# trevor-m/cuda-pathtrace

Measured on AMD Instinct MI355X. Metric: Msamples/s, 9-sphere Cornell box 1024x1024x1024spp, higher is better.
Workload: dtype f32+f64

## Files before the change

### cuda-pathtrace_amd/__init__.py

```python
import ctypes
import os

import numpy as np

_HERE = os.path.dirname(os.path.abspath(__file__))
LIB_PATH = os.environ.get("PT_LIB_OVERRIDE") or os.path.join(_HERE, "libptcore.so")
LAB_LIB_PATH = os.path.join(_HERE, "libptcore_lab.so")
INCLUDE_DIR = os.path.join(os.path.dirname(_HERE), "include")

if not os.path.exists(LIB_PATH):
    raise ImportError(
        f"{LIB_PATH} is missing: build it with `make -C cuda-pathtrace_amd/csrc` "
        "(or __graft_entry__.build()); there is no fallback implementation"
    )

RNG_XORWOW = 0
RNG_PHILOX = 1
CHANNELS = 14

SPHERE_DTYPE = np.dtype([("radius", "<f4"), ("pos", "<f4", 3), ("emission", "<f4", 3), ("color", "<f4", 3)])
assert SPHERE_DTYPE.itemsize == 40


class PtError(RuntimeError):
# ... 115 lines not shown
    "pt_filter_opts_default": (None, [_vp]),
    "pt_filter_create": (ctypes.c_int, [ctypes.c_int, ctypes.c_int, _vp, ctypes.POINTER(_vp)]),
    "pt_filter_destroy": (ctypes.c_int, [_vp]),
    "pt_filter_reserve_frames": (ctypes.c_int, [_vp, ctypes.c_int]),
    "pt_filter_workspace_bytes": (ctypes.c_int, [_vp, ctypes.POINTER(ctypes.c_uint64)]),
    "pt_filter_enqueue": (ctypes.c_int, [_vp, _vp, _vp, ctypes.c_int, _vp, _vp]),
    "pt_filter_run": (ctypes.c_int, [_vp, _vp, _vp, ctypes.c_int, _vp, _fp]),
    "pt_filter_enqueue_frames": (ctypes.c_int, [_vp, ctypes.c_int, _vp, ctypes.c_size_t, _vp, ctypes.c_size_t, ctypes.c_int, _vp]),
    "pt_filter_run_frames": (ctypes.c_int, [_vp, ctypes.c_int, _vp, ctypes.c_size_t, _vp, ctypes.c_size_t, ctypes.c_int, _fp]),
    "pt_progressive_create": (ctypes.c_int, [_vp, ctypes.POINTER(_vp)]),
    "pt_progressive_reset": (ctypes.c_int, [_vp]),
    "pt_progressive_enqueue": (ctypes.c_int, [_vp, ctypes.c_int, _vp, _vp, ctypes.c_int, _fp, _fp, _vp]),
    "pt_progressive_render": (ctypes.c_int, [_vp, ctypes.c_int, _vp, _vp, ctypes.c_int, _fp, _fp, _fp]),
    "pt_progressive_samples": (ctypes.c_int, [_vp, ctypes.POINTER(ctypes.c_int64)]),
    "pt_progressive_variant": (ctypes.c_int, [_vp, ctypes.c_int, ctypes.POINTER(ctypes.c_int)]),
    "pt_progressive_destroy": (ctypes.c_int, [_vp]),
    "pt_progressive_set_adaptive": (ctypes.c_int, [_vp, _vp]),
    "pt_progressive_active": (ctypes.c_int, [_vp, ctypes.POINTER(ctypes.c_int64)]),
    "pt_progressive_counts": (ctypes.c_int, [_vp, _vp, _vp]),
}
LAB_ABI = {
    "pt_debug_unary_map": (ctypes.c_int, [ctypes.c_int, _vp, _vp, ctypes.c_size_t]),
    "pt_debug_unary_compare": (ctypes.c_int, [ctypes.c_int, ctypes.c_int, ctypes.c_uint32, ctypes.c_uint64,
                                              ctypes.POINTER(ctypes.c_uint64), ctypes.POINTER(ctypes.c_uint32)]),
    "pt_debug_div_compare": (ctypes.c_int, [ctypes.c_uint32, ctypes.c_uint32, ctypes.c_uint32, ctypes.c_uint64,
                                            ctypes.POINTER(ctypes.c_uint64), ctypes.POINTER(ctypes.c_uint32),
                                            ctypes.POINTER(ctypes.c_uint32)]),
    "pt_debug_grid_header": (ctypes.c_int, [_vp, ctypes.c_int, ctypes.POINTER(ctypes.c_uint32)]),
    "pt_debug_grid_image": (ctypes.c_int, [_vp, ctypes.c_int, _fp, ctypes.c_int, ctypes.POINTER(ctypes.c_uint32), ctypes.c_size_t,
                                           ctypes.POINTER(ctypes.c_uint64)]),
    "pt_debug_policy_ms": (ctypes.c_int, [ctypes.c_int, ctypes.c_int, ctypes.c_double, ctypes.c_int, ctypes.c_int, ctypes.POINTER(ctypes.c_double)]),
    "pt_debug_policy_choice": (ctypes.c_int, [ctypes.c_int, ctypes.c_double, ctypes.c_int, ctypes.c_int, ctypes.c_int, ctypes.c_int, ctypes.POINTER(ctypes.c_int)]),
    "pt_debug_renderer_batch_launches": (ctypes.c_int, [_vp, ctypes.POINTER(ctypes.c_uint32)]),
    "pt_debug_denoiser_layer_info": (ctypes.c_int, [_vp, ctypes.c_int, ctypes.POINTER(ctypes.c_int), ctypes.POINTER(ctypes.c_int),
                                                    ctypes.c_char_p, ctypes.c_size_t]),
    "pt_debug_denoiser_activation": (ctypes.c_int, [_vp, ctypes.c_int, _vp, ctypes.c_size_t]),
    "pt_debug_denoiser_set_activation": (ctypes.c_int, [_vp, ctypes.c_int, _vp, ctypes.c_size_t]),
    "pt_debug_denoiser_conv_info": (ctypes.c_int, [_vp, ctypes.c_int, ctypes.POINTER(ctypes.c_int), ctypes.POINTER(ctypes.c_int),
                                                   ctypes.c_char_p, ctypes.c_size_t]),
    "pt_debug_denoiser_run_conv": (ctypes.c_int, [_vp, ctypes.c_int, _vp]),
    "pt_debug_denoiser_memory": (ctypes.c_int, [_vp, ctypes.c_int, ctypes.POINTER(ctypes.c_uint64)]),
    "pt_debug_denoiser_last_enqueue": (ctypes.c_int, [_vp, ctypes.POINTER(ctypes.c_int), ctypes.POINTER(ctypes.c_int)]),
    "pt_debug_denoiser_conv_plan": (ctypes.c_int, [_vp, ctypes.c_int, ctypes.c_int, ctypes.POINTER(ctypes.c_int)]),
    "pt_debug_filter_step": (ctypes.c_int, [_vp, _vp, _vp, ctypes.c_int, _vp, ctypes.c_int]),
    "pt_debug_filter_tiled": (ctypes.c_int, [_vp, ctypes.c_int]),
    "pt_debug_progressive_set_samples": (ctypes.c_int, [_vp, ctypes.c_int64]),
    "pt_debug_progressive_record": (ctypes.c_int, [_vp, _vp]),
    "pt_debug_progressive_set_active": (ctypes.c_int, [_vp, _vp]),
}

FN_INV_SQRT_LITERAL, FN_INV_SQRT_FAST, FN_SQRT_LITERAL, FN_SQRT_FAST, FN_SIN, FN_COS, FN_UNIFORM = range(7)
FN_ONEMINUS_LITERAL, FN_ONEMINUS_FAST, FN_ONEMINUS_F32, FN_ONEMINUS_F32_FLAG, FN_ZERO = 7, 8, 9, 10, 11
FN_UNIFORM_LITERAL = 12
FN_SIN_LITERAL, FN_COS_LITERAL = 13, 14

lib = ctypes.CDLL(LIB_PATH)
for _name, (_res, _args) in ABI.items():
    if os.environ.get("PT_LIB_OVERRIDE") and not hasattr(lib, _name):
        continue
    _fn = getattr(lib, _name)
    _fn.restype = _res
    _fn.argtypes = _args
IS_LAB = hasattr(lib, "pt_debug_unary_map")
if IS_LAB:
    for _name, (_res, _args) in LAB_ABI.items():
        _fn = getattr(lib, _name)
# ... 172 lines not shown
    raw = (ctypes.c_uint32 * (int(lay[0]) // 4))()
    eye_c = (ctypes.c_float * 3)(*eye) if eye is not None else None
    check(lib.pt_debug_grid_image(d_scene.ptr, n, eye_c, threads, raw, int(lay[0]), lay))
    u = np.frombuffer(raw, dtype=np.uint32).copy()
    f, b = u.view(np.float32), u.view(np.uint8)
    hdr = {"valid": int(u[0]), "dims": (int(u[1]), int(u[2]), int(u[3])), "origin": (float(f[4]), float(f[5]), float(f[6])),
           "cell_size": float(f[7]), "slack": float(f[9]), "centre": (float(f[10]), float(f[11]), float(f[12])), "far2": float(f[13]),
           "n_big": int(u[14]) & 0xFFFF, "n_entries": int(u[14]) >> 16, "n_items": int(u[15]), "r_small": float(f[16]),
           "r_big": float(f[17]), "max_entries": int(lay[7])}
    if not hdr["valid"]:
        return hdr
    ncells = hdr["dims"][0] * hdr["dims"][1] * hdr["dims"][2]
    u16 = lambda off, cnt: b[off:off + 2 * cnt].view(np.uint16).astype(np.int64)
    hdr["big"] = u16(int(lay[1]), hdr["n_big"])
    start = u16(int(lay[2]), ncells + 1)
    items = u16(int(lay[3]), hdr["n_items"])
    hdr["cells"] = [items[start[c]:start[c + 1]] for c in range(ncells)]
    tab = b[int(lay[4]):int(lay[4]) + 8 * hdr["n_entries"]].view(np.uint32).reshape(-1, 2)
    pooled = []
    for c in range(ncells):
        got, e = [], c
        for _ in range(hdr["n_entries"] + 1):
            w0, w1 = int(tab[e, 0]), int(tab[e, 1])
            k, link = w0 >> 30, (w0 >> 16) & 0x1FFF
            got += [w0 & 0xFFFF, w1 & 0xFFFF, w1 >> 16][:k]
            if link == 0:
                break
            e = link
        pooled.append(np.asarray(got, dtype=np.int64))
    hdr["pooled"] = pooled
    return hdr


def upload_scene(spheres):
    spheres = np.ascontiguousarray(spheres, dtype=SPHERE_DTYPE)
    return DeviceBuffer(max(spheres.nbytes, 4)).upload(spheres), len(spheres)


class Renderer:

    def __init__(self, width, height, spp, threads_per_block=8, *, max_bounces=5, rng_mode=RNG_XORWOW, seed=0,
                 row_begin=0, row_end=0, persist_rng=True, variant=None, layout=LAYOUT_INTERLEAVED, fast_math=False, chunks=0):
        o = RendererOpts()
        lib.pt_renderer_opts_default(ctypes.byref(o))
        o.max_bounces, o.rng_mode, o.seed = max_bounces, rng_mode, seed
        o.row_begin, o.row_end = row_begin, row_end
        o.persist_rng = 1 if persist_rng else 0
        o.layout = layout
        o.fast_math = 1 if fast_math else 0
        o.chunks = chunks
        if variant is not None:
            o.variant = variant
        self.variant = o.variant
        h = _vp()
        check(lib.pt_renderer_create(width, height, spp, threads_per_block, ctypes.byref(o), ctypes.byref(h)))
        self.handle = h.value
        self.width, self.height, self.spp = width, height, spp
        self.row_begin = row_begin
        self.row_end = row_end if (row_begin or row_end) else height
        self.rows = self.row_end - self.row_begin

    @property
    def tile_floats(self):
        return self.rows * self.width * CHANNELS

    def render(self, d_out, d_spheres, n_spheres, basis, eye=DEFAULT_EYE):
# ... 521 lines not shown
```

### cuda-pathtrace_amd/csrc/pt_debug.hip

```cpp
#include "pt_device.h"
#include "pt_internal.h"
#include "pt_kernel.h"
#include "../../include/ptcore_lab.h"

#pragma clang fp contract(off)

namespace pt {

__device__ __forceinline__ float eval_unary(int fn, float x) {
  float s, c;
  switch (fn) {
    case PT_FN_INV_SQRT_LITERAL: return 1.0f / sqrtf(x);
    case PT_FN_INV_SQRT_FAST: return inv_sqrt_spec(x);
    case PT_FN_SQRT_LITERAL: return sqrtf(x);
    case PT_FN_SQRT_FAST: return sqrt_cr_f32(x);
    case PT_FN_SIN: pt_sincos(x, s, c); return s;
    case PT_FN_COS: pt_sincos(x, s, c); return c;
    case PT_FN_UNIFORM: return uniform_from_u32(__float_as_uint(x));
    case PT_FN_ONEMINUS_LITERAL: return (float)sqrt(1.0 - (double)(x * x));
    case PT_FN_ONEMINUS_FAST: return (float)sqrt_cr(1.0 - (double)(x * x));
    case PT_FN_ONEMINUS_F32: {
      bool bad = false;
      const float v = oneminus_f32_nb(x, bad);
      return bad ? (float)sqrt(1.0 - (double)(x * x)) : v;
// ... 96 lines not shown
  return PT_OK;
}

extern "C" int pt_debug_div_compare(uint32_t n_first, uint32_t n_count, uint32_t first_bits, uint64_t count, uint64_t* n_mismatch,
                                    uint32_t* example_bits, uint32_t* example_n) {
  if (!n_mismatch || count > (1ull << 32) || n_first < 1 || n_count < 1 || n_count > 4096)
    return pt_fail(PT_EINVAL, "pt_debug_div_compare: bad arguments");
  unsigned long long* d = nullptr;
  PT_HIPD(hipMalloc((void**)&d, 24));
  PT_HIPD(hipMemset(d, 0, 24));
  hipLaunchKernelGGL(pt::div_compare_kernel, dim3(16384), dim3(256), 0, 0, n_first, n_count, first_bits, count, d);
  hipError_t e = hipGetLastError();
  unsigned long long h[3] = {0, 0, 0};
  if (e == hipSuccess) e = hipMemcpy(h, d, 24, hipMemcpyDeviceToHost);
  (void)hipFree(d);
  if (e != hipSuccess) return pt_fail(PT_EHIP, "pt_debug_div_compare: %s", hipGetErrorString(e));
  *n_mismatch = h[0];
  if (example_bits) *example_bits = (uint32_t)h[1];
  if (example_n) *example_n = (uint32_t)h[2];
  return PT_OK;
}

extern "C" int pt_debug_grid_header(const pt_sphere* d_spheres, int n_spheres, uint32_t header_out[16]) {
  if (!d_spheres || !header_out || n_spheres < 1) return pt_fail(PT_EINVAL, "pt_debug_grid_header: bad arguments");
  uint32_t* d = nullptr;
  PT_HIPD(hipMalloc((void**)&d, pt_kernel_accel_bytes()));
  hipError_t e = pt_launch_build_grid(d_spheres, n_spheres, d, nullptr, true, nullptr);
  if (e == hipSuccess) e = hipMemcpy(header_out, d, 64, hipMemcpyDeviceToHost);
  (void)hipFree(d);
  PT_HIPD(e);
  return PT_OK;
}

extern "C" int pt_debug_grid_image(const pt_sphere* d_spheres, int n_spheres, const float* eye, int threads, uint32_t* image_out,
                                   size_t image_bytes, uint64_t layout_out[8]) {
  if (!d_spheres || !layout_out || n_spheres < 1) return pt_fail(PT_EINVAL, "pt_debug_grid_image: bad arguments");
  pt_kernel_grid_layout(n_spheres, threads, layout_out);
  const size_t need = (size_t)layout_out[0];
  if (!image_out) return PT_OK;
  if (image_bytes < need) return pt_fail(PT_EINVAL, "pt_debug_grid_image: the image needs %zu bytes", need);
  uint32_t* d = nullptr;
  PT_HIPD(hipMalloc((void**)&d, need));
  hipError_t e = hipMemset(d, 0, need);
  if (e == hipSuccess) e = pt_launch_build_grid(d_spheres, n_spheres, d, eye, true, nullptr, threads);
  if (e == hipSuccess) e = hipMemcpy(image_out, d, need, hipMemcpyDeviceToHost);
  (void)hipFree(d);
  PT_HIPD(e);
  return PT_OK;
}
```

### cuda-pathtrace_amd/csrc/pt_grid.h

```cpp
#pragma once
#include "pt_intersect.h"

#pragma clang fp contract(off)

namespace pt {

#ifndef PT_V13_LAST_SHORTCUT
#define PT_V13_LAST_SHORTCUT 1
#endif
#ifndef PT_GRID_MAX_CELLS
#define PT_GRID_MAX_CELLS 4096
#endif
#ifndef PT_GRID_CELLS_PER_SPHERE
#define PT_GRID_CELLS_PER_SPHERE 2.75f
#endif
#ifndef PT_GRID_EXACT_REG
#define PT_GRID_EXACT_REG 1
#endif
constexpr int kGridMaxCells = PT_GRID_MAX_CELLS;
#ifndef PT_GRID_TESTS_PER_TRIP
#define PT_GRID_TESTS_PER_TRIP 3
#endif
#ifndef PT_GRID_MAX_ITEMS
#define PT_GRID_MAX_ITEMS 8192
#endif
constexpr int kGridMaxItems = PT_GRID_MAX_ITEMS;
constexpr int kGridMaxBig = 64;
constexpr int kGridMaxSpheres = PT_GRID_MAX_SPHERES;
constexpr int kGridBuildThreads = 1024;

struct GridHeader {
  uint32_t valid, nx, ny, nz;
  float ox, oy, oz, cs;
  float inv_cs, slack, cx, cy;
  float cz, far2;
  uint32_t n_big, n_items;
  float r_small, r_big;
  uint32_t prim_base, n_emis;
};
static_assert(sizeof(GridHeader) == 80, "GridHeader layout");

constexpr int kGridMaxEntries = 8191;
constexpr size_t kGridBigOff = sizeof(GridHeader);
constexpr size_t kGridStartOff = kGridBigOff + kGridMaxBig * sizeof(uint16_t);
constexpr size_t kGridItemsOff = kGridStartOff + (kGridMaxCells + 2) * sizeof(uint16_t);
constexpr size_t kGridCellsOff = (kGridItemsOff + kGridMaxItems * sizeof(uint16_t) + 7) & ~(size_t)7;
constexpr int kGridMaxEmis = 32;
constexpr int kGridEmisWords = PT_GRID_MAX_SPHERES / 32 + kGridMaxEmis / 2;
constexpr size_t kGridEmisOff = kGridCellsOff + (size_t)(kGridMaxEntries + 1) * 2 * sizeof(uint32_t);
constexpr size_t kGridAccelBytes = kGridEmisOff + (size_t)kGridEmisWords * sizeof(uint32_t);

constexpr int kPoolLdsTarget = 80 * 1024;
constexpr int kPoolRing = 512;
constexpr int kPoolWaveBytes = kPoolRing * 4 + 64 * 8 + 64 * 4 + 64 * 4 + 16;
constexpr int kGridBigGeomBytes = kGridMaxBig * (int)sizeof(float4);
constexpr int kPrimEntriesPerLane = 2;
constexpr int kPrimMaxList = 5;
__host__ __device__ inline int grid_prim_entries(int threads) { return threads * kPrimEntriesPerLane; }
__host__ __device__ inline int grid_lds_target(int threads) { return threads > PT_GRID_BLOCK_THREADS ? 2 * kPoolLdsTarget - 2048 : kPoolLdsTarget; }
__host__ __device__ inline int grid_max_entries(int n, bool pooled, int threads = PT_GRID_BLOCK_THREADS) {
  if (!pooled) return kGridMaxEntries;
  const int prim = grid_prim_entries(threads);
  const int fixed = kTablesF4 * (int)sizeof(float4) + (threads / 64) * kPoolWaveBytes + kGridBigGeomBytes +
                    kGridMaxBig * (int)sizeof(uint16_t) + 32 + prim * 8 + kGridEmisWords * 4;
  int avail = grid_lds_target(threads) - fixed - n * (int)sizeof(float4);
  if (avail < 8192) avail = 8192;
  const int e = avail / 8;
  return e > kGridMaxEntries - prim ? kGridMaxEntries - prim : e;
}

__host__ __device__ inline size_t grid_lds_bytes(int n, bool pooled, int threads = PT_GRID_BLOCK_THREADS) {
  const size_t head = (size_t)n * sizeof(float4) + kGridBigGeomBytes + kGridMaxBig * sizeof(uint16_t);
  if (pooled) return head + (size_t)(grid_max_entries(n, true, threads) + grid_prim_entries(threads)) * 8 + (size_t)kGridEmisWords * 4;
  return head + (kGridCellsOff - kGridStartOff);
}

struct GridLds {
  bool valid;
  GridHeader h;
  const float4* geom;
  const float4* bigg;
  const uint16_t* big;
  const uint16_t* cell_start;
  const uint16_t* items;
  const uint2* cells;
  const uint32_t* em_bits;
  const uint16_t* em_list;
};

template <bool POOLED>
__device__ __forceinline__ GridLds stage_grid(const pt_sphere* __restrict__ spheres, int n, const uint32_t* __restrict__ accel,
                                              float4* lds) {
  GridLds g;
  g.h = *reinterpret_cast<const GridHeader*>(accel);
  g.valid = g.h.valid != 0u;
  g.geom = lds;
  float4* bigg = lds + n;
  g.bigg = bigg;
  uint32_t* tab = reinterpret_cast<uint32_t*>(bigg + kGridMaxBig);
  g.big = reinterpret_cast<const uint16_t*>(tab);
  const int ncells = (int)(g.h.nx * g.h.ny * g.h.nz);
  uint32_t* after_big = tab + kGridMaxBig / 2;
  g.em_bits = nullptr;
  g.em_list = nullptr;
  uint32_t* em_lds = nullptr;
  if constexpr (POOLED) {
    g.cells = reinterpret_cast<const uint2*>(after_big);
    g.items = nullptr;
    g.cell_start = nullptr;
    em_lds = after_big + 2 * (size_t)(grid_max_entries(n, true, (int)blockDim.x) + grid_prim_entries((int)blockDim.x));
    g.em_bits = em_lds;
    g.em_list = reinterpret_cast<const uint16_t*>(em_lds + PT_GRID_MAX_SPHERES / 32);
  } else {
    g.cell_start = reinterpret_cast<const uint16_t*>(after_big);
    g.items = g.cell_start + (kGridMaxCells + 2);
    g.cells = nullptr;
  }
  if (!g.valid) return g;
  for (int i = threadIdx.x; i < n; i += blockDim.x) {
    const pt_sphere sp = spheres[i];
    lds[i] = make_float4(sp.pos[0], sp.pos[1], sp.pos[2], sp.radius * sp.radius);
  }
  const int n_big = (int)(g.h.n_big & 0xFFFFu);
  for (int i = threadIdx.x; i < n_big; i += blockDim.x) {
    const pt_sphere sp = spheres[reinterpret_cast<const uint16_t*>(accel + kGridBigOff / 4)[i]];
    bigg[i] = make_float4(sp.pos[0], sp.pos[1], sp.pos[2], sp.radius * sp.radius);
  }
  const uint32_t* src = accel + kGridBigOff / 4;
  for (int i = threadIdx.x; i < kGridMaxBig / 2; i += blockDim.x) tab[i] = src[i];
  if constexpr (POOLED) {
    const int n_entries = (int)(g.h.n_big >> 16);
    const uint32_t* src_cells = accel + kGridCellsOff / 4;
    for (int i = threadIdx.x; i < 2 * n_entries; i += blockDim.x) after_big[i] = src_cells[i];
    const uint32_t* src_em = accel + kGridEmisOff / 4;
    for (int i = threadIdx.x; i < kGridEmisWords; i += blockDim.x) em_lds[i] = src_em[i];
  } else {
    const int words_i = ((int)g.h.n_items + 1) / 2;
    const uint32_t* src_items = accel + kGridItemsOff / 4;
    const uint32_t* src_start = accel + kGridStartOff / 4;
    const int words_s = (ncells + 2 + 1) / 2;
    for (int i = threadIdx.x; i < words_s; i += blockDim.x) after_big[i] = src_start[i];
    uint32_t* dst_items = after_big + (kGridMaxCells + 2) / 2;
    for (int i = threadIdx.x; i < words_i; i += blockDim.x) dst_items[i] = src_items[i];
  }
  __syncthreads();
// ... 301 lines not shown
    __syncthreads();
    scan_tmp[tid] = sum;
    __syncthreads();
    for (int off = 1; off < kGridBuildThreads; off <<= 1) {
      const uint32_t u = tid >= off ? scan_tmp[tid - off] : 0u;
      __syncthreads();
      scan_tmp[tid] += u;
      __syncthreads();
    }
    uint32_t run = scan_tmp[tid] - sum;
    n_ext = scan_tmp[kGridBuildThreads - 1];
    uint32_t* cells = accel + kGridCellsOff / 4;
#pragma unroll
    for (int j = 0; j < kPer; j++) {
      const int c = kPer * tid + j;
      if (c < (int)ncells) {
        uint32_t p = cell_start[c], rem = (uint32_t)cell_start[c + 1] - p, idx = (uint32_t)c, next = ncells + run;
        for (;;) {
          const uint32_t k = rem <= 3u ? rem : 2u, link = rem <= 3u ? 0u : next;
          const uint32_t i0 = k > 0u ? items[p] : 0u, i1 = k > 1u ? items[p + 1u] : 0u, i2 = k > 2u ? items[p + 2u] : 0u;
          cells[2 * idx] = i0 | (link << 16) | (k << 30);
          cells[2 * idx + 1] = i1 | (i2 << 16);
          if (link == 0u) break;
          idx = link;
          next++;
          p += 2u;
          rem -= 2u;
        }
      }
      run += v[j];
    }
  }
  if (tid == 0) {
    GridHeader h;
    h.valid = 1u;
    h.nx = nx;
    h.ny = ny;
    h.nz = nz;
    h.ox = lo[0];
    h.oy = lo[1];
    h.oz = lo[2];
    h.cs = cs;
    h.inv_cs = inv;
    h.slack = slack;
    h.cx = ctr[0];
    h.cy = ctr[1];
    h.cz = ctr[2];
    h.far2 = far * far;
    h.n_big = n_big | ((ncells + n_ext) << 16);
    h.n_items = total;
    h.r_small = r_small;
    h.r_big = r_big;
    h.prim_base = (uint32_t)max_entries;
    h.n_emis = s_n_emis > (uint32_t)kGridMaxEmis ? 0xFFFFu : s_n_emis;
    *hdr = h;
  }
}

#ifdef PT_GRID_STATS
__device__ unsigned long long g_grid_stats[8];
__device__ unsigned long long g_grid_hist[4][64];
#define PT_HIST_DECL int hist_tests = 0, hist_steps = 0, hist_trips = 0, hist_rounds = 0
#define PT_HIST_LANE(var, n) do { var += (n); } while (0)
#define PT_HIST_END(in_walk) do { \
    if (in_walk) { atomicAdd(&g_grid_hist[0][hist_tests < 63 ? hist_tests : 63], 1ull); atomicAdd(&g_grid_hist[1][hist_steps < 63 ? hist_steps : 63], 1ull); } \
    if ((threadIdx.x & 63) == __builtin_ctzll(__builtin_amdgcn_ballot_w64(true))) { \
// ... 53 lines not shown
  s.i1 = Te < s.T1 ? i : s.i1;
  s.T2 = __builtin_amdgcn_fmed3f(s.T1, s.T2, Te);
  s.T1 = fminf(s.T1, Te);
}

__device__ __forceinline__ void near2_resolve(Near2& s, uint32_t doubts, const float4 g0, int i0, const float4 g1, int i1,
                                              const float4 g2, int i2, F3 o, F3 d, float a, float Tlim_hi) {
  while (doubts != 0u) {
    const bool k0 = (doubts & 1u) != 0u, k1 = !k0 & ((doubts & 2u) != 0u);
    const float4 g = k0 ? g0 : (k1 ? g1 : g2);
    const int i = k0 ? i0 : (k1 ? i1 : i2);
    near2_exact(s, g, i, o, d, a, Tlim_hi);
    doubts &= k0 ? ~1u : (k1 ? ~2u : ~4u);
  }
}

struct GridWalk {
  Near2 s;
  float a;
  float tmax0, tmax1, tmax2, tdel0, tdel1, tdel2;
  int cidx;
  int cs0, cs1, cs2;
  uint32_t left;
  uint32_t k0, k1;
  uint32_t n0, n1;
  bool have_next;
  bool walking;
  uint32_t e0, e1;
  float t_box;
  bool forced;
  __device__ __forceinline__ bool busy() const { return (k0 < k1) | have_next | walking; }
};

template <bool POOLED = false>
__device__ __forceinline__ void grid_begin(GridWalk& w, const GridLds& G, F3 o, F3 d, float a, bool prim = false, bool last = false) {
  const float INF = __builtin_inff();
  const float two_a = 2.0f * a, a4 = 4.0f * a;
  const float Tlim = 1000000.0f * two_a;
  const float Tlim_hi = Tlim * 1.0000153f;
  w.a = a;
  w.s = Near2{INF, INF, 0};
  {
    const int nb = (int)(G.h.n_big & 0xFFFFu);
    int k = 0;
    for (; k + 2 <= nb; k += 2) {
      const int i = (int)G.big[k], j = (int)G.big[k + 1];
      const float4 gi = G.bigg[k], gj = G.bigg[k + 1];
      const bool di = near2_test<true>(w.s, gi, i, o, d, a4, Tlim_hi);
      const bool dj = near2_test<true>(w.s, gj, j, o, d, a4, Tlim_hi);
      if (__builtin_expect(di | dj, 0)) near2_resolve(w.s, (di ? 1u : 0u) | (dj ? 2u : 0u), gi, i, gj, j, gj, j, o, d, a, Tlim_hi);
    }
    if (k < nb) {
      const int i = (int)G.big[k];
      const float4 gi = G.bigg[k];
      const bool doubt = near2_test<true>(w.s, gi, i, o, d, a4, Tlim_hi);
      if (__builtin_expect(__builtin_amdgcn_ballot_w64(doubt) != 0ull, 0)) {
        if (doubt) near2_exact(w.s, gi, i, o, d, a, Tlim_hi);
      }
    }
  }
  bool settled = false;
#if PT_V13_LAST_SHORTCUT
  if constexpr (POOLED) {
    if (G.h.n_emis != 0xFFFFu && (G.h.n_big & 0xFFFFu) != 0u && __builtin_amdgcn_ballot_w64(last) != 0ull) {
      if (last) {
        const int ne = (int)G.h.n_emis;
        for (int k = 0; k < ne; k++) {
          const int i = (int)G.em_list[k];
          const float4 gi = G.geom[i];
          if (near2_test<true>(w.s, gi, i, o, d, a4, Tlim_hi)) near2_exact(w.s, gi, i, o, d, a, Tlim_hi);
        }
        const uint32_t emits = (G.em_bits[(uint32_t)w.s.i1 >> 5] >> ((uint32_t)w.s.i1 & 31u)) & 1u;
        settled = (w.s.T1 < INF) & (emits == 0u) & (w.s.T2 > w.s.T1 * 1.0000038f) & (w.s.T1 < Tlim * 0.99998f);
      }
    }
  }
#endif
  bool active = false;
  int cidx = 0;
  float t_out = INF;
  w.tmax0 = INF, w.tmax1 = INF, w.tmax2 = INF, w.tdel0 = INF, w.tdel1 = INF, w.tdel2 = INF;
  w.cs0 = 0, w.cs1 = 0, w.cs2 = 0;
  uint32_t left = 0x20080200u;
  const float slack_t = G.h.slack * __builtin_amdgcn_rsqf(a);
  {
  const float gmin[3] = {G.h.ox, G.h.oy, G.h.oz};
  const float dims_f[3] = {(float)G.h.nx, (float)G.h.ny, (float)G.h.nz};
  const int dims[3] = {(int)G.h.nx, (int)G.h.ny, (int)G.h.nz};
  const float oo[3] = {o.x, o.y, o.z}, dd[3] = {d.x, d.y, d.z};
  const float tiny = __builtin_amdgcn_sqrtf(a) * 9.094947e-13f;
  float inv[3], t_in = 0.0f;
// ... 526 lines not shown
            const int j = tc >= tmx ? (int)((tc - tmx) * __builtin_amdgcn_rcpf(td) + 0.75f) : 0;
            const float tj = tmx + (float)j * td;
            return ((tj < tc) | ((tj == tc) & (m < ax))) ? j + 1 : j;
          };
          const int c0 = k0 ? (int)i + 1 : taken(m0, d0, 0), c1 = k1 ? (int)i + 1 : taken(m1, d1, 1),
                    c2 = (k0 | k1) ? taken(m2, d2, 2) : (int)i + 1;
          const int sx = (int)G.h.nx, sxy = (int)(G.h.nx * G.h.ny);
          const int idx = base + ((nn >> 24) & 1u ? -c0 : c0) + ((nn >> 25) & 1u ? -c1 : c1) * sx + ((nn >> 26) & 1u ? -c2 : c2) * sxy;
          const uint32_t at = (uint32_t)idx < last_cell ? (uint32_t)idx : last_cell;
          const uint2 e = G.cells[at];
          se0 = e.x, se1 = e.y;
          tag = (info & 0xFFu) << 16;
          if (PT_DBG_OWNED(info & 0xFFu)) PT_DBG("SERVE helper %d li %u axis %d i %u tc %g c %d %d %d base %d idx %d entry %08x %08x nn %08x\n", lane, li, k0 ? 0 : (k1 ? 1 : 2), i, tc, c0, c1, c2, base, idx, e.x, e.y, nn);
        }
      }
      push(se0, se1, tag, true);
      const bool fin = __builtin_amdgcn_ballot_w64((links != 0u) | (sw_done < sw_total)) == 0;
      drain(fin);
      if (fin) break;
    }
  }
  PT_HIST_END(true);
  const unsigned long long k = __hip_atomic_load(P.key1 + lane, __ATOMIC_RELAXED, __HIP_MEMORY_SCOPE_WORKGROUP);
  walk.s.T1 = __uint_as_float((uint32_t)(k >> 32));
  walk.s.i1 = walk.s.T1 < INF ? (int)(uint32_t)k : 0;
  walk.s.T2 = __uint_as_float(__hip_atomic_load(P.t2 + lane, __ATOMIC_RELAXED, __HIP_MEMORY_SCOPE_WORKGROUP));
  if (PT_DBG_ME()) PT_DBG("FINAL T1 %g i1 %d T2 %g forced %d swept %d\n", walk.s.T1, walk.s.i1, walk.s.T2, (int)walk.forced, (int)sweep);
}

__device__ __forceinline__ bool intersect_scene_grid_pooled(const SceneLds& sc, const GridLds& G, int n, F3 o, F3 d, float a,
                                                            float& t_hit, int& idx, bool walker = true, bool prim = false,
                                                            bool last = false) {
  GridWalk w;
  grid_begin<true>(w, G, o, d, a, prim & walker, last & walker);
  const float INF = __builtin_inff();
  w.s.T1 = walker ? w.s.T1 : INF;
  w.s.T2 = walker ? w.s.T2 : INF;
  w.walking = w.walking & walker;
  w.e0 = walker ? w.e0 : 0u;
  w.e1 = walker ? w.e1 : 0u;
  grid_trips_pooled(w, G, pool_of_wave(sc.pool), o, d);
  if (!walker) return false;
  return grid_end(w, sc, G, n, o, d, t_hit, idx);
}

__device__ __forceinline__ bool intersect_scene_v13(const SceneLds& sc, int n, F3 o, F3 d, float& t_hit, int& idx, bool live = true,
                                                    bool prim = false, bool last = false) {
  if (n <= 0) return false;
  const float a = dot(d, d);
  const GridLds& G = *sc.grid;
  if (G.valid) {
    const bool admitted = live && grid_admits(G, o, d, a);
    PT_STATW(7, __builtin_amdgcn_ballot_w64(live & !admitted) != 0 ? 1 : 0);
    const bool walk_here = __builtin_amdgcn_ballot_w64(admitted) != 0;
    if (admitted | (walk_here & !live)) {
      const bool hit = intersect_scene_grid_pooled(sc, G, n, o, d, a, t_hit, idx, admitted, prim, last);
      if (admitted) return hit;
    }
  }
  if (!live) return false;
  return intersect_scene_screened_large(sc, n, o, d, make_ray_const(d), t_hit, idx);
}

}
```

### cuda-pathtrace_amd/csrc/pt_kernel.h

```cpp
#pragma once
#include <hip/hip_runtime.h>
#include <stddef.h>
#include <stdint.h>

#include "../../include/ptcore.h"

#ifndef PT_BLOCK_THREADS
#define PT_BLOCK_THREADS 256
#endif
#ifndef PT_PRIO_MIN_SPP
#define PT_PRIO_MIN_SPP 512
#endif
#ifndef PT_PRIO_MIN_SPP_REGEN
#define PT_PRIO_MIN_SPP_REGEN 32
#endif
#ifndef PT_FOOTPRINT_MIN_SPP
#define PT_FOOTPRINT_MIN_SPP 8
#endif
#ifndef PT_SCREEN_UNROLL
#define PT_SCREEN_UNROLL 9
#endif
#define PT_VARIANT_AUTO (-1)
#define PT_DEFAULT_VARIANT 6
#ifndef PT_SCREEN_MAX_SPHERES
// ... 163 lines not shown
size_t pt_kernel_lds_bytes(int n_spheres, int variant);
int pt_kernel_max_spheres(int variant);
hipError_t pt_launch_pixel_kernel(const PixelKernelArgs& a, int rng_mode, int variant, hipStream_t stream);
bool pt_kernel_has_frames(int variant, int n_spheres, int max_bounces, bool planar);
hipError_t pt_launch_frames_kernel(const FramesKernelArgs& fa, int rng_mode, int variant, hipStream_t stream);
bool pt_kernel_has_resume(int variant);
const void* pt_resume_kernel_symbol(int rng_mode, int variant, int n_spheres, int max_bounces, bool planar);
hipError_t pt_launch_resume_kernel(const ResumeKernelArgs& ra, int rng_mode, int variant, hipStream_t stream);
const void* pt_adaptive_kernel_symbol(int rng_mode, int variant, int n_spheres, int max_bounces, bool planar);
hipError_t pt_launch_adaptive_kernel(const AdaptiveKernelArgs& aa, int rng_mode, int variant, hipStream_t stream);
struct AdaptiveState {
  uint32_t* counts;
  uint32_t* list;
  uint8_t* mask;
  uint32_t* block_sums;
  uint32_t* words;
};
struct AdaptiveRule {
  double tolerance;
  double floor;
  int32_t min_samples;
  int32_t radius;
};
#define PT_ADAPTIVE_BLOCK 256
#define PT_ADAPTIVE_MAX_RADIUS 4
hipError_t pt_launch_adaptive_select(const AdaptiveState& s, const AdaptiveRule& rule, const uint32_t* rec, uint32_t tile_pixels,
                                     int width, int n, int n_end, int mode, bool peek, hipStream_t stream);
hipError_t pt_launch_adaptive_finalize(const uint32_t* rec, const uint32_t* counts, float* out, uint32_t tile_pixels, bool planar,
                                       hipStream_t stream);
hipError_t pt_launch_build_grid(const pt_sphere* spheres, int n, uint32_t* accel, const float* eye ,
                                bool pooled , hipStream_t stream,
                                int threads = PT_GRID_BLOCK_THREADS );
void pt_kernel_grid_layout(int n_spheres, int threads, uint64_t out[8]);
size_t pt_kernel_accel_bytes(void);
hipError_t pt_launch_setup_random(uint32_t* state, int width, int row_begin, uint32_t tile_pixels, uint64_t seed,
                                  hipStream_t stream);
const void* pt_fast_kernel_symbol(int rng_mode, int n_spheres, int max_bounces);
size_t pt_fast_kernel_lds_bytes(int n_spheres);
hipError_t pt_launch_fast_kernel(const PixelKernelArgs& a, int rng_mode, hipStream_t stream);
```

### cuda-pathtrace_amd/csrc/pt_kernel.hip

```cpp
#include "pt_trace.h"

#pragma clang fp contract(off)

static constexpr int kNumVariants = 15;
static constexpr int kT = PT_BLOCK_THREADS, kTG = PT_GRID_BLOCK_THREADS, kTW = PT_GRID_WIDE_THREADS;
static constexpr int kW = PT_MIN_WAVES, kWG = PT_GRID_MIN_WAVES, kWD = PT_GRID12_MIN_WAVES, kWP = PT_POOL_MIN_WAVES;
static constexpr VariantInfo kVariants[kNumVariants] = {
     {true,  1, kT,  PT_LEAN_NEVER,  PT_LDS_PLAIN,  PT_GRID_NONE,   false, false, false, false, PT_CHUNK_NONE,     false, kW,   PT_LOOP_SAMPLES,   0,     0},
     {false, 1, kT,  PT_LEAN_NEVER,  PT_LDS_PLAIN,  PT_GRID_NONE,   false, false, false, false, PT_CHUNK_NONE,     false, kW,   PT_LOOP_SAMPLES,   1,     1},
     {false, 1, kT,  PT_LEAN_NEVER,  PT_LDS_PLAIN,  PT_GRID_NONE,   false, false, false, false, PT_CHUNK_NONE,     false, kW,   PT_LOOP_SAMPLES,   2,     2},
     {false, 1, kT,  PT_LEAN_NEVER,  PT_LDS_PACKED, PT_GRID_NONE,   false, false, false, false, PT_CHUNK_NONE,     false, kW,   PT_LOOP_SAMPLES,   3,     3},
     {false, 1, kT,  PT_LEAN_NEVER,  PT_LDS_PLAIN,  PT_GRID_NONE,   false, false, false, false, PT_CHUNK_NONE,     false, kW,   PT_LOOP_SAMPLES,   4,     4},
     {false, 1, kT,  PT_LEAN_NEVER,  PT_LDS_PLAIN,  PT_GRID_NONE,   false, false, false, false, PT_CHUNK_NONE,     false, kW,   PT_LOOP_SAMPLES,   5,     5},
     {true,  1, kT,  PT_LEAN_BIG,    PT_LDS_WALLS,  PT_GRID_NONE,   false, true,  true,  true,  PT_CHUNK_ONE_LANE, true,  kW,   PT_LOOP_SAMPLES,   6,     6},
     {false, 1, kT,  PT_LEAN_NEVER,  PT_LDS_PLAIN,  PT_GRID_NONE,   false, false, false, false, PT_CHUNK_NONE,     false, kW,   PT_LOOP_PAIRS,     6,     7},
     {true,  4, kT,  PT_LEAN_BIG,    PT_LDS_PLAIN,  PT_GRID_NONE,   false, true,  false, false, PT_CHUNK_SPLIT,    true,  0,    PT_LOOP_SAMPLES,   6,     8},
     {true,  2, kT,  PT_LEAN_NEVER,  PT_LDS_PLAIN,  PT_GRID_NONE,   false, true,  false, false, PT_CHUNK_SPLIT,    true,  0,    PT_LOOP_SAMPLES,   6,     9},
     {true,  1, kT,  PT_LEAN_BIG,    PT_LDS_PLAIN,  PT_GRID_NONE,   false, false, true,  false, PT_CHUNK_NONE,     false, kW,   PT_LOOP_REGEN,     6,     10},
     {false, 1, kTG, PT_LEAN_ALWAYS, PT_LDS_PLAIN,  PT_GRID_LANE,   false, false, false, false, PT_CHUNK_NONE,     false, kWG,  PT_LOOP_REGEN,     11,    11},
     {false, 1, kTG, PT_LEAN_ALWAYS, PT_LDS_PLAIN,  PT_GRID_LANE,   false, false, false, false, PT_CHUNK_NONE,     false, kWD,  PT_LOOP_DECOUPLED, 11,    12},
     {true,  1, kTG, PT_LEAN_ALWAYS, PT_LDS_PLAIN,  PT_GRID_POOLED, false, false, true,  false, PT_CHUNK_GRID,     true,  kWP,  PT_LOOP_REGEN,     13,    13},
     {true,  1, kTW, PT_LEAN_ALWAYS, PT_LDS_PLAIN,  PT_GRID_POOLED, true,  false, true,  false, PT_CHUNK_GRID,     false, kWP,  PT_LOOP_REGEN,     13,    13},
};
static constexpr VariantInfo kNoVariant = {false, 1, kT, PT_LEAN_NEVER, PT_LDS_PLAIN, PT_GRID_NONE, false, false, false, false, PT_CHUNK_NONE, false, kW, PT_LOOP_SAMPLES, 0, 0};
// ... 973 lines not shown
  return (const void*)select_kernel<>(rng_mode, run_variant(variant, max_bounces), n_spheres, max_bounces, planar);
}
const void* pt_resume_kernel_symbol(int rng_mode, int variant, int n_spheres, int max_bounces, bool planar) {
  return (const void*)select_kernel<false, true>(rng_mode, variant, n_spheres, max_bounces, planar);
}
const void* pt_adaptive_kernel_symbol(int rng_mode, int variant, int n_spheres, int max_bounces, bool planar) {
  return (const void*)select_kernel<false, true, true>(rng_mode, variant, n_spheres, max_bounces, planar);
}

#ifdef PT_SCREEN_STATS
extern "C" int pt_debug_screen_stats(unsigned long long out[8], int reset) {
  unsigned long long zero[8] = {0, 0, 0, 0, 0, 0, 0, 0};
  if (hipMemcpyFromSymbol(out, HIP_SYMBOL(pt::g_screen_stats), sizeof(zero)) != hipSuccess) return -2;
  if (reset && hipMemcpyToSymbol(HIP_SYMBOL(pt::g_screen_stats), zero, sizeof(zero)) != hipSuccess) return -2;
  return 0;
}
#endif

#ifdef PT_GRID_STATS
extern "C" int pt_debug_grid_hist(unsigned long long out[256], int reset) {
  static unsigned long long zero[256];
  if (hipMemcpyFromSymbol(out, HIP_SYMBOL(pt::g_grid_hist), sizeof(zero)) != hipSuccess) return -2;
  if (reset && hipMemcpyToSymbol(HIP_SYMBOL(pt::g_grid_hist), zero, sizeof(zero)) != hipSuccess) return -2;
  return 0;
}
extern "C" int pt_debug_grid_stats(unsigned long long out[8], int reset) {
  unsigned long long zero[8] = {0, 0, 0, 0, 0, 0, 0, 0};
  if (hipMemcpyFromSymbol(out, HIP_SYMBOL(pt::g_grid_stats), sizeof(zero)) != hipSuccess) return -2;
  if (reset && hipMemcpyToSymbol(HIP_SYMBOL(pt::g_grid_stats), zero, sizeof(zero)) != hipSuccess) return -2;
  return 0;
}
#endif

size_t pt_kernel_accel_bytes(void) { return pt::kGridAccelBytes; }

int pt_kernel_max_spheres(int variant) {
  const VariantInfo& v = pt_kernel_variant(variant);
  if (v.lean != PT_LEAN_NEVER) return 1 << 26;
  const size_t fixed = tail_lds_bytes(0, v) + pt::kTablesF4 * sizeof(float4);
  if (v.lds_extra == PT_LDS_PACKED) return (int)((PT_LDS_BUDGET_BYTES - fixed - 2 * sizeof(float4)) / (5 * sizeof(float4)));
  return (int)((PT_LDS_BUDGET_BYTES - fixed) / (4 * sizeof(float4)));
}

hipError_t pt_launch_build_grid(const pt_sphere* spheres, int n, uint32_t* accel, const float* eye, bool pooled, hipStream_t stream, int threads) {
  hipLaunchKernelGGL(pt::build_grid_kernel, dim3(1), dim3(pt::kGridBuildThreads), 0, stream, spheres, n, accel, eye ? eye[0] : 0.0f,
                     eye ? eye[1] : 0.0f, eye ? eye[2] : 0.0f, eye ? 1 : 0, pt::grid_max_entries(n, pooled, threads));
  return hipGetLastError();
}

void pt_kernel_grid_layout(int n_spheres, int threads, uint64_t out[8]) {
  out[0] = pt::kGridAccelBytes;
  out[1] = pt::kGridBigOff;
  out[2] = pt::kGridStartOff;
  out[3] = pt::kGridItemsOff;
  out[4] = pt::kGridCellsOff;
  out[5] = pt::kGridEmisOff;
  out[6] = (uint64_t)pt::kGridMaxCells;
  out[7] = (uint64_t)pt::grid_max_entries(n_spheres, true, threads);
}

bool pt_kernel_chunked(int variant, int n_spheres, int max_bounces, bool planar, int spp, uint32_t chunks) {
  const VariantInfo& v = pt_kernel_variant(variant);
  const bool build_chunks = v.chunk_build(!lds_lean(n_spheres, v) && ref_config(n_spheres, max_bounces, v, planar));
  return build_chunks && chunks > 1u && chunks <= (uint32_t)PT_CHUNKS_MAX && spp >= 2 * (int)chunks &&
         (spp + (int)chunks - 1) / (int)chunks <= (v.chunk_family == PT_CHUNK_GRID ? PT_CHUNK_MAX_SAMPLES_GRID : PT_CHUNK_MAX_SAMPLES);
}
// ... 99 lines not shown
```

### cuda-pathtrace_amd/csrc/pt_walls.h

```cpp
#pragma once
#include <math.h>
#include "../../include/ptcore.h"

namespace pt {

struct WallLayout {
  int obj[3];
  int minus[3];
  int plus[3];
  bool ok;
};

__host__ __device__ inline WallLayout classify_walls(const pt_sphere* s, int n) {
  WallLayout w{{6, 7, 8}, {0, 2, 4}, {1, 3, 5}, false};
  const WallLayout none = w;
  if (n != 9) return w;
  double rmax = 0.0;
  for (int i = 0; i < 9; i++) {
    const double r = (double)s[i].radius;
    if (!(r >= 0.0) || !(r < 1e30)) return none;
    rmax = r > rmax ? r : rmax;
  }
  int walls[6], objs[3], nw = 0, no = 0;
  for (int i = 0; i < 9; i++) {
// ... 22 lines not shown
    const double r = (double)sw.radius;
    if (sw.emission[0] != 0.0f || sw.emission[1] != 0.0f || sw.emission[2] != 0.0f) return none;
    if (!(r >= 100.0 * ext) || !(r > 0.0)) return none;
    double off[3];
    int ax = 0;
    for (int k = 0; k < 3; k++) {
      off[k] = (double)sw.pos[k] - p[k];
      if (!(fabs(off[k]) < 1e30)) return none;
      if (fabs(off[k]) > fabs(off[ax])) ax = k;
    }
    if (!(fabs(off[ax]) >= 0.5 * r)) return none;
    for (int k = 0; k < 3; k++)
      if (k != ax && !(fabs(off[k]) <= 1e-2 * r)) return none;
    int* slot = off[ax] > 0.0 ? &pl[ax] : &mi[ax];
    if (*slot >= 0) return none;
    *slot = walls[j];
  }
  for (int k = 0; k < 3; k++) {
    if (mi[k] < 0 || pl[k] < 0) return none;
    const pt_sphere &a = s[pl[k]], &b = s[mi[k]];
    if (!((double)a.pos[k] - (double)a.radius < (double)b.pos[k] + (double)b.radius)) return none;
    for (int j = 0; j < 3; j++)
      if (j != k && __builtin_bit_cast(unsigned, a.pos[j]) != __builtin_bit_cast(unsigned, b.pos[j])) return none;
  }
  for (int k = 0; k < 3; k++) {
    w.obj[k] = objs[k];
    w.minus[k] = mi[k];
    w.plus[k] = pl[k];
  }
  w.ok = true;
  return w;
}

}
```

### include/ptcore_lab.h

```cpp
#ifndef PTCORE_LAB_H
#define PTCORE_LAB_H

#include "ptcore.h"

#ifdef __cplusplus
extern "C" {
#endif

enum {
  PT_FN_INV_SQRT_LITERAL = 0,
  PT_FN_INV_SQRT_FAST = 1,
  PT_FN_SQRT_LITERAL = 2,
  PT_FN_SQRT_FAST = 3,
  PT_FN_SIN = 4,
  PT_FN_COS = 5,
  PT_FN_UNIFORM = 6,
  PT_FN_ONEMINUS_LITERAL = 7,
  PT_FN_ONEMINUS_FAST = 8,
  PT_FN_ONEMINUS_F32 = 9,
  PT_FN_ONEMINUS_F32_FLAG = 10,
  PT_FN_ZERO = 11,
  PT_FN_UNIFORM_LITERAL = 12,
  PT_FN_SIN_LITERAL = 13,
  PT_FN_COS_LITERAL = 14,
  PT_FN_COUNT = 15
};
int pt_debug_unary_map(int fn, const float* d_in, float* d_out, size_t n);
int pt_debug_unary_compare(int fn_a, int fn_b, uint32_t first_bits, uint64_t count, uint64_t* n_mismatch,
                           uint32_t* example_bits);
int pt_debug_div_compare(uint32_t n_first, uint32_t n_count, uint32_t first_bits, uint64_t count, uint64_t* n_mismatch,
                         uint32_t* example_bits, uint32_t* example_n);
int pt_debug_grid_header(const pt_sphere* d_spheres, int n_spheres, uint32_t header_out[16]);
int pt_debug_grid_image(const pt_sphere* d_spheres, int n_spheres, const float* eye, int threads, uint32_t* image_out,
                        size_t image_bytes, uint64_t layout_out[8]);
int pt_debug_policy_ms(int rng_mode, int variant, double waves_per_simd, int spp, int bounces, double* ms);
int pt_debug_policy_choice(int rng_mode, double waves_per_simd, int spp, int bounces, int with9, int chunked, int* variant);
int pt_debug_renderer_batch_launches(pt_renderer* r, uint32_t* launches);

int pt_debug_denoiser_layer_info(pt_denoiser* d, int layer, int* n_layers, int shape[3], char* name, size_t name_len);
int pt_debug_denoiser_activation(pt_denoiser* d, int layer, float* h_out, size_t n_floats);
int pt_debug_denoiser_set_activation(pt_denoiser* d, int layer, const float* h_in, size_t n_floats);
int pt_debug_denoiser_conv_info(pt_denoiser* d, int conv, int* n_convs, int info[12], char* name, size_t name_len);
int pt_debug_denoiser_run_conv(pt_denoiser* d, int conv, float* d_rgb);
int pt_debug_denoiser_memory(pt_denoiser* d, int layer, uint64_t info[6]);
int pt_debug_denoiser_last_enqueue(pt_denoiser* d, int* groups, int* launches);
int pt_debug_denoiser_conv_plan(pt_denoiser* d, int n_frames, int conv, int info[6]);

int pt_debug_filter_step(pt_filter* f, float* d_frame, float* d_rgb, int samples, const uint32_t* d_counts, int step);
int pt_debug_filter_tiled(pt_filter* f, int on);

int pt_debug_progressive_set_samples(pt_progressive* p, int64_t samples);
int pt_debug_progressive_record(pt_progressive* p, uint32_t* host);
int pt_debug_progressive_set_active(pt_progressive* p, const uint8_t* host_mask);

#ifdef __cplusplus
}
#endif
#endif
```

Before: 24430.

## Test only the facing Cornell-box wall per axis in pooled grid traversal

When grid building detects six huge walls forming an axis-aligned box, it reorders them into the first six big-sphere slots and sets a flag in the accel buffer. During pooled grid traversal the ray then tests only the wall it faces on each axis, using a cheap certificate that it starts inside the far wall and that wall cannot be hit sooner. If any lane in the wavefront fails the certificate, the behind walls are tested too. This cuts big-sphere intersection tests from six to about three per ray, at the cost of more detection logic and ballots.

```diff
diff --git a/cuda-pathtrace_amd/__init__.py b/cuda-pathtrace_amd/__init__.py
--- a/cuda-pathtrace_amd/__init__.py
+++ b/cuda-pathtrace_amd/__init__.py
@@ -171,6 +171,7 @@
     "pt_debug_policy_ms": (ctypes.c_int, [ctypes.c_int, ctypes.c_int, ctypes.c_double, ctypes.c_int, ctypes.c_int, ctypes.POINTER(ctypes.c_double)]),
     "pt_debug_policy_choice": (ctypes.c_int, [ctypes.c_int, ctypes.c_double, ctypes.c_int, ctypes.c_int, ctypes.c_int, ctypes.c_int, ctypes.POINTER(ctypes.c_int)]),
     "pt_debug_renderer_batch_launches": (ctypes.c_int, [_vp, ctypes.POINTER(ctypes.c_uint32)]),
+    "pt_debug_grid_wall_calls": (ctypes.c_int, [ctypes.POINTER(ctypes.c_uint64), ctypes.c_int]),
     "pt_debug_denoiser_layer_info": (ctypes.c_int, [_vp, ctypes.c_int, ctypes.POINTER(ctypes.c_int), ctypes.POINTER(ctypes.c_int),
                                                     ctypes.c_char_p, ctypes.c_size_t]),
     "pt_debug_denoiser_activation": (ctypes.c_int, [_vp, ctypes.c_int, _vp, ctypes.c_size_t]),
@@ -409,6 +410,12 @@
     return hdr
 
 
+def grid_wall_calls(reset=False):
+    c = (ctypes.c_uint64 * 2)()
+    check(lib.pt_debug_grid_wall_calls(c, 1 if reset else 0))
+    return int(c[0]), int(c[1])
+
+
 def upload_scene(spheres):
     spheres = np.ascontiguousarray(spheres, dtype=SPHERE_DTYPE)
     return DeviceBuffer(max(spheres.nbytes, 4)).upload(spheres), len(spheres)
diff --git a/cuda-pathtrace_amd/csrc/pt_debug.hip b/cuda-pathtrace_amd/csrc/pt_debug.hip
--- a/cuda-pathtrace_amd/csrc/pt_debug.hip
+++ b/cuda-pathtrace_amd/csrc/pt_debug.hip
@@ -152,6 +152,15 @@
   return PT_OK;
 }
 
+extern "C" int pt_debug_grid_wall_calls(uint64_t calls[2], int reset) {
+  if (!calls) return pt_fail(PT_EINVAL, "pt_debug_grid_wall_calls: NULL argument");
+  unsigned long long got[2] = {0, 0};
+  PT_HIPD(pt_kernel_grid_wall_calls(got, reset != 0));
+  calls[0] = got[0];
+  calls[1] = got[1];
+  return PT_OK;
+}
+
 extern "C" int pt_debug_grid_image(const pt_sphere* d_spheres, int n_spheres, const float* eye, int threads, uint32_t* image_out,
                                    size_t image_bytes, uint64_t layout_out[8]) {
   if (!d_spheres || !layout_out || n_spheres < 1) return pt_fail(PT_EINVAL, "pt_debug_grid_image: bad arguments");
diff --git a/cuda-pathtrace_amd/csrc/pt_grid.h b/cuda-pathtrace_amd/csrc/pt_grid.h
--- a/cuda-pathtrace_amd/csrc/pt_grid.h
+++ b/cuda-pathtrace_amd/csrc/pt_grid.h
@@ -48,7 +48,8 @@
 constexpr int kGridMaxEmis = 32;
 constexpr int kGridEmisWords = PT_GRID_MAX_SPHERES / 32 + kGridMaxEmis / 2;
 constexpr size_t kGridEmisOff = kGridCellsOff + (size_t)(kGridMaxEntries + 1) * 2 * sizeof(uint32_t);
-constexpr size_t kGridAccelBytes = kGridEmisOff + (size_t)kGridEmisWords * sizeof(uint32_t);
+constexpr size_t kGridWallOff = kGridEmisOff + (size_t)kGridEmisWords * sizeof(uint32_t);
+constexpr size_t kGridAccelBytes = kGridWallOff + 4 * sizeof(uint32_t);
 
 constexpr int kPoolLdsTarget = 80 * 1024;
 constexpr int kPoolRing = 512;
@@ -86,6 +87,7 @@
   const uint2* cells;
   const uint32_t* em_bits;
   const uint16_t* em_list;
+  uint32_t walls;
 };
 
 template <bool POOLED>
@@ -103,6 +105,7 @@
   uint32_t* after_big = tab + kGridMaxBig / 2;
   g.em_bits = nullptr;
   g.em_list = nullptr;
+  g.walls = 0u;
   uint32_t* em_lds = nullptr;
   if constexpr (POOLED) {
     g.cells = reinterpret_cast<const uint2*>(after_big);
@@ -111,6 +114,7 @@
     em_lds = after_big + 2 * (size_t)(grid_max_entries(n, true, (int)blockDim.x) + grid_prim_entries((int)blockDim.x));
     g.em_bits = em_lds;
     g.em_list = reinterpret_cast<const uint16_t*>(em_lds + PT_GRID_MAX_SPHERES / 32);
+    if (g.valid) g.walls = accel[kGridWallOff / 4];
   } else {
     g.cell_start = reinterpret_cast<const uint16_t*>(after_big);
     g.items = g.cell_start + (kGridMaxCells + 2);
@@ -478,6 +482,24 @@
     }
   }
   if (tid == 0) {
+    uint32_t walls_ok = 0u;
+    const GridWalls gw = classify_grid_walls(spheres, big, (int)n_big);
+    if (gw.ok) {
+      uint16_t want[6];
+      for (int k = 0; k < 3; k++) {
+        want[2 * k] = big[gw.minus[k]];
+        want[2 * k + 1] = big[gw.plus[k]];
+      }
+      for (int j = 0; j < 6; j++) {
+        int p = j;
+        while (big[p] != want[j]) p++;
+        const uint16_t t = big[j];
+        big[j] = big[p];
+        big[p] = t;
+      }
+      walls_ok = 1u;
+    }
+    accel[kGridWallOff / 4] = walls_ok;
     GridHeader h;
     h.valid = 1u;
     h.nx = nx;
@@ -597,8 +619,58 @@
   __device__ __forceinline__ bool busy() const { return (k0 < k1) | have_next | walking; }
 };
 
+#if PT_BUILD_EXPERIMENTS
+__device__ unsigned long long g_grid_wall_calls[2];
+#endif
+template <int AX>
+__device__ __forceinline__ bool near2_wall_pair(Near2& s, const GridLds& G, F3 o, F3 d, float a4, float Tlim_hi, float& bB, bool& inB) {
+  const float dk = AX == 0 ? d.x : AX == 1 ? d.y : d.z;
+  const int f = 2 * AX + (dk < 0.0f ? 1 : 0);
+  const float4 gf = G.bigg[f], gb = G.bigg[f ^ 1];
+  const F3 off = mk3(o.x - gf.x, o.y - gf.y, o.z - gf.z);
+  const F3 offb = with_axis<AX>(off, (AX == 0 ? o.x : AX == 1 ? o.y : o.z) - (AX == 0 ? gb.x : AX == 1 ? gb.y : gb.z));
+  bB = 2.0f * dot(d, offb);
+  inB = neg_finite(fmaf(gb.w, 5.9837103e-08f, dot(offb, offb) - gb.w));
+  return near2_test<true>(s, gf, (int)G.big[f], o, d, a4, Tlim_hi);
+}
+__device__ __forceinline__ void near2_walls(Near2& s, const GridLds& G, F3 o, F3 d, float a, float a4, float Tlim_hi, bool walker) {
+  float b0, b1, b2;
+  bool in0, in1, in2;
+  const bool f0 = near2_wall_pair<0>(s, G, o, d, a4, Tlim_hi, b0, in0);
+  const bool f1 = near2_wall_pair<1>(s, G, o, d, a4, Tlim_hi, b1, in1);
+  const bool f2 = near2_wall_pair<2>(s, G, o, d, a4, Tlim_hi, b2, in2);
+  uint32_t doubts = (f0 ? 1u : 0u) | (f1 ? 2u : 0u) | (f2 ? 4u : 0u);
+  const float K = s.T1 * 1.0009765625f;
+  const bool cert = (neg_finite(fmaf(2.0f, b0, K)) & in0) & (neg_finite(fmaf(2.0f, b1, K)) & in1) & (neg_finite(fmaf(2.0f, b2, K)) & in2);
+  const bool fallback = __builtin_amdgcn_ballot_w64(walker & !cert) != 0ull;
+#if PT_BUILD_EXPERIMENTS
+  if (__builtin_amdgcn_ballot_w64(walker) != 0ull && (threadIdx.x & 63) == __builtin_ctzll(__builtin_amdgcn_ballot_w64(true)))
+    atomicAdd(&g_grid_wall_calls[fallback ? 1 : 0], 1ull);
+#endif
+  auto wall_at = [&](int ax, bool behind) {
+    const float dk = ax == 0 ? d.x : ax == 1 ? d.y : d.z;
+    return (2 * ax + (dk < 0.0f ? 1 : 0)) ^ (behind ? 1 : 0);
+  };
+  if (__builtin_expect(fallback, 0)) {
+#pragma unroll
+    for (int ax = 0; ax < 3; ax++) {
+      const int p = wall_at(ax, true);
+      if (near2_test<true>(s, G.bigg[p], (int)G.big[p], o, d, a4, Tlim_hi)) doubts |= 8u << ax;
+    }
+  }
+  if (__builtin_expect(__builtin_amdgcn_ballot_w64(doubts != 0u) != 0ull, 0)) {
+    while (doubts != 0u) {
+      const int k = __builtin_ctz(doubts);
+      const int p = wall_at(k >= 3 ? k - 3 : k, k >= 3);
+      near2_exact(s, G.bigg[p], (int)G.big[p], o, d, a, Tlim_hi);
+      doubts &= doubts - 1u;
+    }
+  }
+}
+
 template <bool POOLED = false>
-__device__ __forceinline__ void grid_begin(GridWalk& w, const GridLds& G, F3 o, F3 d, float a, bool prim = false, bool last = false) {
+__device__ __forceinline__ void grid_begin(GridWalk& w, const GridLds& G, F3 o, F3 d, float a, bool prim = false, bool last = false,
+                                           bool walker = true) {
   const float INF = __builtin_inff();
   const float two_a = 2.0f * a, a4 = 4.0f * a;
   const float Tlim = 1000000.0f * two_a;
@@ -608,6 +680,9 @@
   {
     const int nb = (int)(G.h.n_big & 0xFFFFu);
     int k = 0;
+    bool walled = false;
+    if constexpr (POOLED) walled = G.walls != 0u;
+    if (walled) k = 6;
     for (; k + 2 <= nb; k += 2) {
       const int i = (int)G.big[k], j = (int)G.big[k + 1];
       const float4 gi = G.bigg[k], gj = G.bigg[k + 1];
@@ -622,6 +697,9 @@
       if (__builtin_expect(__builtin_amdgcn_ballot_w64(doubt) != 0ull, 0)) {
         if (doubt) near2_exact(w.s, gi, i, o, d, a, Tlim_hi);
       }
+    }
+    if constexpr (POOLED) {
+      if (walled) near2_walls(w.s, G, o, d, a, a4, Tlim_hi, walker);
     }
   }
   bool settled = false;
@@ -1214,7 +1292,7 @@
                                                             float& t_hit, int& idx, bool walker = true, bool prim = false,
                                                             bool last = false) {
   GridWalk w;
-  grid_begin<true>(w, G, o, d, a, prim & walker, last & walker);
+  grid_begin<true>(w, G, o, d, a, prim & walker, last & walker, walker);
   const float INF = __builtin_inff();
   w.s.T1 = walker ? w.s.T1 : INF;
   w.s.T2 = walker ? w.s.T2 : INF;
diff --git a/cuda-pathtrace_amd/csrc/pt_kernel.h b/cuda-pathtrace_amd/csrc/pt_kernel.h
--- a/cuda-pathtrace_amd/csrc/pt_kernel.h
+++ b/cuda-pathtrace_amd/csrc/pt_kernel.h
@@ -219,6 +219,9 @@
                                 bool pooled , hipStream_t stream,
                                 int threads = PT_GRID_BLOCK_THREADS );
 void pt_kernel_grid_layout(int n_spheres, int threads, uint64_t out[8]);
+#if PT_BUILD_EXPERIMENTS
+hipError_t pt_kernel_grid_wall_calls(unsigned long long calls[2], bool reset);
+#endif
 size_t pt_kernel_accel_bytes(void);
 hipError_t pt_launch_setup_random(uint32_t* state, int width, int row_begin, uint32_t tile_pixels, uint64_t seed,
                                   hipStream_t stream);
diff --git a/cuda-pathtrace_amd/csrc/pt_kernel.hip b/cuda-pathtrace_amd/csrc/pt_kernel.hip
--- a/cuda-pathtrace_amd/csrc/pt_kernel.hip
+++ b/cuda-pathtrace_amd/csrc/pt_kernel.hip
@@ -1029,6 +1029,16 @@
 }
 #endif
 
+#if PT_BUILD_EXPERIMENTS
+hipError_t pt_kernel_grid_wall_calls(unsigned long long calls[2], bool reset) {
+  const unsigned long long zero[2] = {0, 0};
+  hipError_t e = hipDeviceSynchronize();
+  if (e == hipSuccess) e = hipMemcpyFromSymbol(calls, HIP_SYMBOL(pt::g_grid_wall_calls), sizeof(zero));
+  if (e == hipSuccess && reset) e = hipMemcpyToSymbol(HIP_SYMBOL(pt::g_grid_wall_calls), zero, sizeof(zero));
+  return e;
+}
+#endif
+
 size_t pt_kernel_accel_bytes(void) { return pt::kGridAccelBytes; }
 
 int pt_kernel_max_spheres(int variant) {
diff --git a/cuda-pathtrace_amd/csrc/pt_walls.h b/cuda-pathtrace_amd/csrc/pt_walls.h
--- a/cuda-pathtrace_amd/csrc/pt_walls.h
+++ b/cuda-pathtrace_amd/csrc/pt_walls.h
@@ -78,4 +78,68 @@
   return w;
 }
 
+struct GridWalls {
+  int minus[3], plus[3];
+  bool ok;
+};
+
+__host__ __device__ inline GridWalls classify_grid_walls(const pt_sphere* s, const unsigned short* outside, int n_out) {
+  GridWalls w{{-1, -1, -1}, {-1, -1, -1}, false};
+  const GridWalls none = w;
+  if (n_out < 6 || n_out > 64) return none;
+  double rmax = 0.0;
+  for (int i = 0; i < n_out; i++) {
+    const double r = (double)s[outside[i]].radius;
+    if (!(r >= 0.0) || !(r < 1e30)) return none;
+    rmax = r > rmax ? r : rmax;
+  }
+  int walls[6], nw = 0;
+  for (int i = 0; i < n_out; i++)
+    if ((double)s[outside[i]].radius >= 0.5 * rmax) {
+      if (nw == 6) return none;
+      walls[nw++] = i;
+    }
+  if (nw != 6) return none;
+  double p[3] = {0.0, 0.0, 0.0};
+  for (int j = 0; j < 6; j++)
+    for (int k = 0; k < 3; k++) p[k] += (double)s[outside[walls[j]]].pos[k] / 6.0;
+  double ext = 0.0;
+  for (int i = 0; i < n_out; i++) {
+    if ((double)s[outside[i]].radius >= 0.5 * rmax) continue;
+    for (int k = 0; k < 3; k++) {
+      const double e = fabs((double)s[outside[i]].pos[k] - p[k]);
+      if (!(e < 1e30)) return none;
+      ext = e > ext ? e : ext;
+    }
+  }
+  for (int j = 0; j < 6; j++) {
+    const pt_sphere& sw = s[outside[walls[j]]];
+    const double r = (double)sw.radius;
+    if (sw.emission[0] != 0.0f || sw.emission[1] != 0.0f || sw.emission[2] != 0.0f) return none;
+    if (!(r >= 100.0 * ext) || !(r > 0.0)) return none;
+    double off[3];
+    int ax = 0;
+    for (int k = 0; k < 3; k++) {
+      off[k] = (double)sw.pos[k] - p[k];
+      if (!(fabs(off[k]) < 1e30)) return none;
+      if (fabs(off[k]) > fabs(off[ax])) ax = k;
+    }
+    if (!(fabs(off[ax]) >= 0.5 * r)) return none;
+    for (int k = 0; k < 3; k++)
+      if (k != ax && !(fabs(off[k]) <= 1e-2 * r)) return none;
+    int* slot = off[ax] > 0.0 ? &w.plus[ax] : &w.minus[ax];
+    if (*slot >= 0) return none;
+    *slot = walls[j];
+  }
+  for (int k = 0; k < 3; k++) {
+    if (w.minus[k] < 0 || w.plus[k] < 0) return none;
+    const pt_sphere &a = s[outside[w.plus[k]]], &b = s[outside[w.minus[k]]];
+    if (!((double)a.pos[k] - (double)a.radius < (double)b.pos[k] + (double)b.radius)) return none;
+    for (int j = 0; j < 3; j++)
+      if (j != k && __builtin_bit_cast(unsigned, a.pos[j]) != __builtin_bit_cast(unsigned, b.pos[j])) return none;
+  }
+  w.ok = true;
+  return w;
 }
+
+}
diff --git a/include/ptcore_lab.h b/include/ptcore_lab.h
--- a/include/ptcore_lab.h
+++ b/include/ptcore_lab.h
@@ -36,6 +36,7 @@
 int pt_debug_policy_ms(int rng_mode, int variant, double waves_per_simd, int spp, int bounces, double* ms);
 int pt_debug_policy_choice(int rng_mode, double waves_per_simd, int spp, int bounces, int with9, int chunked, int* variant);
 int pt_debug_renderer_batch_launches(pt_renderer* r, uint32_t* launches);
+int pt_debug_grid_wall_calls(uint64_t calls[2], int reset);
 
 int pt_debug_denoiser_layer_info(pt_denoiser* d, int layer, int* n_layers, int shape[3], char* name, size_t name_len);
 int pt_debug_denoiser_activation(pt_denoiser* d, int layer, float* h_out, size_t n_floats);
```

Measured after the change: 24450, median of 3. No clear change (+0.1%).
